# klemens-floege/oneprot

Measured on AMD Instinct MI355X. Metric: protein-pairs/sec/node (seq+struct-token, L=512, ESM-2-150M), higher is better.
Workload: dtype bf16; 1 GPU; cfg-2: seq<->struct_token sub-step, facebook/esm2_t30_150M_UR50D / facebook/esm2_t30_150M_UR50D, L=512, 256 pairs/GPU per modality, global batch 256, output_dim 1024, CLIP local_loss+gather_with_grad, L1 0.01, Adam 1e-3, clip 1.0, sequence encoder frozen (reference default), random-init weights; global_batch=256, seq_len=512, parallelism=dp1, frozen_sequence_encoder=True

## Files before the change

include/oneprot_hip.h:

```cpp
#ifndef ONEPROT_HIP_H
#define ONEPROT_HIP_H
#include <stddef.h>
#include <stdint.h>
#ifdef __cplusplus
extern "C" {
#endif

int oneprot_abi_version(void);

int oneprot_esm_embed_fwd(const int64_t* ids, const float* table, float* x, float* row_scale, int B, int L, int d, int vocab,
                          int pad_id, int mask_id, int token_dropout, void* stream);
size_t oneprot_esm_embed_bwd_workspace(int T, int d, int vocab);
int oneprot_esm_embed_bwd(const int64_t* ids, const float* dx, const float* row_scale, float* dtable, void* workspace, int B, int L, int d,
                          int vocab, int pad_id, int mask_id, int token_dropout, int accumulate, void* stream);
int oneprot_bert_embed_fwd(const int64_t* ids, const float* word, const float* pos, const float* type0, const float* gamma, const float* beta,
                           float* x_f32, void* x_bf16, int B, int L, int d, int vocab, float eps, void* stream);

int oneprot_layernorm_fwd(const void* x, int x_is_bf16, const float* gamma, const float* beta, void* y_bf16, float* y_f32, float* mean,
                          float* rstd, int64_t T, int d, float eps, void* stream);
size_t oneprot_layernorm_bwd_workspace(int d);
int oneprot_layernorm_bwd(const void* dy, int dy_mode, const float* wrow, int L, const void* x, int x_is_bf16, const float* gamma,
                          const float* mean, const float* rstd, const float* add_to, float* dx, void* dx_bf16 ,
                          float* dgamma, float* dbeta, void* workspace, int64_t T, int d, int accumulate_param_grads, void* stream);
int oneprot_lnpool_fwd(const float* x, const int64_t* ids, int pad_id, const float* gamma, const float* beta, float* pooled, float* mean,
                       float* rstd, float* wrow, void* hidden_bf16, float* hidden_f32, int B, int L, int d, float eps, int mode, void* stream);

int oneprot_pool_fwd(const float* x, const int64_t* ids, int pad_id, float* pooled, int B, int L, int d, int mode, void* stream);
int oneprot_pool_bwd(const float* dpooled, const int64_t* ids, int pad_id, float* g, void* g_bf16, int B, int L, int d, int mode, void* stream);
int oneprot_embed_scatter_sorted(const float* dx, const int64_t* perm, const int64_t* seg_start, const int64_t* seg_row, int64_t n_tokens, int n_seg,
                                 int d, int skip_row, float* dtable, void* stream);
int oneprot_rowsum_f32(const float* x, float* out, int R, int64_t n, void* stream);

int oneprot_attnpool_fwd(const float* x, const int64_t* ids, int pad_id, const float* w, const float* bias, float* pooled, float* attn, int B, int L,
                         int d, void* stream);
size_t oneprot_attnpool_bwd_workspace(int B, int d);
int oneprot_attnpool_bwd(const float* x, const float* attn, const float* w, const float* dpooled, float* dw, float* db, float* dx, void* workspace,
                         int B, int L, int d, void* stream);

enum {
  ONEPROT_EPI_BF16 = 0,
  ONEPROT_EPI_F32 = 1,
  ONEPROT_EPI_BIAS_GELU = 2,
  ONEPROT_EPI_BIAS_RESID = 3,
  ONEPROT_EPI_QKV_ROPE = 4,
  ONEPROT_EPI_GELU_BWD = 5
};
int oneprot_gemm_bf16_nt(const void* A, const void* Bw, int64_t M, int N, int K, int lda, int ldb, int epilogue, const float* bias,
                         void* out0, void* out1, void* out2, const void* aux, const float* rope_cos, const float* rope_sin, float q_scale,
                         int L, int H, int hd, void* stream);
int oneprot_gemm_ln_pack_weight(const void* W_bf16 , void* Wp, int N, int K, void* stream);
int oneprot_gemm_bf16_nt_resid_ln(const void* A, const void* Wp, int64_t M, int N, int K, int lda, const float* bias, const float* resid, float* x_out,
                                  const float* gamma, const float* beta, float eps, void* h_out, float* mean, float* rstd, void* stream);
size_t oneprot_sched_workspace_bytes(int64_t M_max);
int oneprot_alloc_uncached(void** out, size_t bytes);
int oneprot_free_uncached(void* ptr);
int oneprot_sched_workspace_init(void* sched_ws, size_t bytes, void* stream);
void oneprot_dynamic_tiles(void* sched_ws, size_t bytes);
int oneprot_sched_late_draws(const void* sched_ws);
int64_t oneprot_sched_epoch(const void* sched_ws);
int oneprot_gemm_resid_ln8_eligible(int64_t M, int N, int K);
int oneprot_gemm_resid_ln8_error(const void* sched_ws);
int oneprot_gemm_resid_ln8_error_clear(void* sched_ws, void* stream);
void oneprot_gemm_resid_ln8_poll_bound(int polls);
int oneprot_gemm_bf16_nt_resid_ln8(const void* A, const void* W, int64_t M, int N, int K, int lda, int ldb, const float* bias, const float* resid,
                                   float* x_out, const float* gamma, const float* beta, float eps, void* h_bf16, float* stats, void* sched_ws,
                                   size_t sched_ws_bytes, void* stream);
void oneprot_gemm_ln_form(int form);
int oneprot_gemm_ln_form_get(void);
void oneprot_gemm_force_shape(int shape);
void oneprot_gemm_tune(int sup_m, int sup_n);
size_t oneprot_gemm_bf16_tn_workspace(int N, int K);
void oneprot_gemm_tn_variant(int v);
void oneprot_cu_reserve(int cus);
int oneprot_gemm_bf16_tn(const void* dY, const void* X, int64_t M, int N, int K, int ldy, int ldx, float* dW, float* dbias, void* workspace,
                         size_t workspace_bytes, int accumulate, void* stream);
int oneprot_sgemm(const float* A, const float* B, float* C, int M, int N, int K, int transA, int b_is_kn, float alpha, int accumulate, void* stream);

int oneprot_attn_fwd(const void* q, const void* k, const void* v, const float* key_bias, void* ctx, float* lse, int B, int H, int L, int hd,
                     void* stream);
size_t oneprot_attn_bwd_workspace(int B, int H, int L);
int oneprot_attn_bwd(const void* q, const void* k, const void* v, const float* key_bias, const void* ctx, const void* dctx, const float* lse,
                     const float* rope_cos, const float* rope_sin, float q_scale, void* dqkv, void* workspace, int B, int H, int L, int hd,
                     void* stream);
int oneprot_attn_fwd_dropout(const void* q, const void* k, const void* v, const float* key_bias, void* ctx, float* lse, int B, int H, int L, int hd,
                             float p, uint64_t seed, uint64_t stream_id, void* stream);
int oneprot_attn_bwd_dropout(const void* q, const void* k, const void* v, const float* key_bias, const void* ctx, const void* dctx, const float* lse,
                             const float* rope_cos, const float* rope_sin, float q_scale, void* dqkv, void* workspace, int B, int H, int L, int hd,
                             float p, uint64_t seed, uint64_t stream_id, void* stream);
int oneprot_attn_dropout_keep(void* keep, int B, int H, int L, float p, uint64_t seed, uint64_t stream_id, void* stream);
void oneprot_attn_force_bwd_path(int path);
void oneprot_attn_force_fwd_path(int path);

int oneprot_gelu_f32(const float* x, float* y, int64_t n, void* stream);
int oneprot_gelu_bwd_f32(const float* x, const float* dy, float* dx, int64_t n, void* stream);
int oneprot_l2norm_fwd(const float* x, float* y, float* inv_norm, int R, int D, float scale, void* stream);
int oneprot_l2norm_bwd(const float* y, const float* dy, const float* inv_norm, float* dx, int R, int D, float scale, float l1_coef, void* stream);
int oneprot_ce_fwd_bwd(float* logits, float* loss_sum, float* row_loss_ws , int R, int C, int label_offset, float row_weight, void* stream);
int oneprot_siglip_fwd_bwd(float* logits, float* loss_sum, float* row_loss_ws , int B, float logit_bias, int negative_only, void* stream);
int oneprot_siglip_fwd_bwd_dev(float* logits, float* loss_sum, float* row_loss_ws , int B, const float* logit_bias_dev, int negative_only, void* stream);
int oneprot_diag_rank(const float* logits, int* rank_row, int* rank_col, int N, void* stream);
int oneprot_abs_sum(const float* x, float* out_sum, void* workspace , int64_t n, float coef, void* stream);

int oneprot_dot_f32(const float* x, const float* y, float* out_sum, void* workspace , int64_t n, float coef, void* stream);

int oneprot_l1_bwd(const float* x, float* dx, int64_t n, float coef, const float* upstream, int accumulate, void* stream);
int oneprot_scale_by_device_scalar(float* x, int64_t n, const float* s, void* stream);
int oneprot_key_padding_bias(const int64_t* ids, float* bias, int64_t n, int pad_id, void* stream);

int oneprot_dropout_bf16(const void* x, void* y, int64_t n, float p, uint64_t seed, uint64_t stream_id, void* stream);
int oneprot_dropout_f32(const float* x, float* y, int64_t n, float p, uint64_t seed, uint64_t stream_id, void* stream);
int oneprot_dropout_add_f32(const float* x, const float* resid, float* y, int64_t n, float p, uint64_t seed, uint64_t stream_id, void* stream);
int oneprot_dropout_add_layernorm_fwd(const float* x, const float* resid, float* s_out, const float* gamma, const float* beta, void* y_bf16, float* y_f32,
                                      float* mean, float* rstd, int64_t T, int d, float eps, float p, uint64_t seed, uint64_t stream_id, void* stream);
int oneprot_dropout_bwd_add_bf16(const void* dy, void* dx, int64_t n, float p, uint64_t seed, uint64_t stream_id, void* stream);
int oneprot_dropout_bwd_add_f32(const void* dy, float* dx, int64_t n, float p, uint64_t seed, uint64_t stream_id, void* stream);

size_t oneprot_sumsq_workspace(void);
int oneprot_sumsq(const float* x, int64_t n, float* sumsq, void* workspace, void* stream);
int oneprot_clip_coef(const float* sumsq, float max_norm, float* coef, float* norm_out, const void* sched_ws , void* stream);
int oneprot_adam_step(float* p, const float* g, float* m, float* v, int64_t n, float lr, float beta1, float beta2, float eps, float weight_decay,
                      int step, const float* grad_scale, void* stream);

int oneprot_cast_f32_to_bf16(const float* src, void* dst, int64_t n, void* stream);
int oneprot_transpose_cast_f32_to_bf16(const float* src, void* dst, int R, int C, void* stream);
int oneprot_transpose_cast_f32_to_bf16_batched(const float* src, void* dst, int R, int C, int64_t src_stride, int64_t dst_stride, int count, void* stream);
size_t oneprot_colsum_workspace(int N);
// ... 28 lines not shown
```

oneprot_amd/csrc/gemm_tn.hip:

```cpp
#include "common.h"
#include "../../include/oneprot_hip.h"

#define TN_MAX_SLAB_TILES 512

static __device__ __attribute__((aligned(16))) unsigned int g_zero_page[4] = {0, 0, 0, 0};

__device__ __forceinline__ int tn_f(int r) { return 2 * ((r & 3) | (((r >> 3) & 1) << 2)); }

__device__ __forceinline__ bf8_t tn_frag(const unsigned char* tile, int mb, int c0, int lane) {
  const int g = lane >> 4, i = lane & 15;
  const int r0 = mb + 8 * g + (i >> 2), r1 = r0 + 4;
  const int col = c0 + 4 * (i & 3);
  const int chunk = col >> 3, within = (col & 7) * 2;
  const unsigned char* p0 = tile + r0 * 256 + ((chunk ^ tn_f(r0)) << 4) + within;
  const unsigned char* p1 = tile + r1 * 256 + ((chunk ^ tn_f(r1)) << 4) + within;
  const s16x4 a = __builtin_amdgcn_ds_read_tr16_b64_v4i16((__attribute__((address_space(3))) s16x4*)p0);
  const s16x4 b = __builtin_amdgcn_ds_read_tr16_b64_v4i16((__attribute__((address_space(3))) s16x4*)p1);
  s16x8 o;
  o[0] = a[0]; o[1] = a[1]; o[2] = a[2]; o[3] = a[3]; o[4] = b[0]; o[5] = b[1]; o[6] = b[2]; o[7] = b[3];
  return __builtin_bit_cast(bf8_t, o);
}

template <int N> __device__ __forceinline__ void tn_wait_vmcnt() { asm volatile("s_waitcnt vmcnt(%0)" ::"n"(N) : "memory"); }

template <int BT, int NSTAGE, int MINW, bool RS>
__global__ void __launch_bounds__(256, MINW) k_gemm_tn(const bf16_t* __restrict__ dY, const bf16_t* __restrict__ X, int M, int N, int K, int ldy, int ldx,
                                                       float* __restrict__ slab, float* __restrict__ bias_slab, int tiles_k, int tiles_all, int S, int m_per_split) {
  constexpr int TILE_BYTES = BT * 256;
  constexpr int STAGE_BYTES = 2 * TILE_BYTES;
  constexpr int IPW = BT / 4 / 4;
  constexpr int LPS = 2 * IPW;
  extern __shared__ __attribute__((aligned(16))) unsigned char smem[];
  const int per_xcd = gridDim.x >> 3;
  const int xcd = blockIdx.x & 7, seq = blockIdx.x >> 3;
  const int w = xcd * per_xcd + seq;
  if (w >= tiles_all * S) return;
  const int split = w / tiles_all, tile = w - split * tiles_all;
  const int tn = tile / tiles_k, tk = tile - tn * tiles_k;
  const int n0 = tn * 128, k0 = tk * 128;
  const int tid = threadIdx.x, lane = tid & 63;
  const int wave = __builtin_amdgcn_readfirstlane(tid >> 6);
  const int wr = wave >> 1, wc = wave & 1;
  const int mbeg = split * m_per_split;
  const int mend = min(M, mbeg + m_per_split);
  const int nsteps = (mend - mbeg + BT - 1) / BT;

  const int srow = lane >> 4, schunk = lane & 15;
  const unsigned char* zero = reinterpret_cast<const unsigned char*>(g_zero_page);
  int rows[IPW], ycol_ok[IPW], xcol_ok[IPW];
  size_t yoff[IPW], xoff[IPW];
#pragma unroll
  for (int i = 0; i < IPW; ++i) {
    rows[i] = (wave * IPW + i) * 4 + srow;
    const int sc = schunk ^ tn_f(rows[i]);
// ... 157 lines not shown
        if (n < N) bias_slab[(size_t)split * N + n] = accb[i][r];
      }
  }
}

__global__ void __launch_bounds__(256) k_tn_reduce(const float* __restrict__ slab, float* __restrict__ dW, size_t n4, size_t stride4, int S, int accumulate,
                                                   const float* __restrict__ bias_slab, float* __restrict__ db, int N, int bias_blocks) {
  const int wblocks = (int)gridDim.x - bias_blocks;
  if ((int)blockIdx.x >= wblocks) {
    const int n = ((int)blockIdx.x - wblocks) * 256 + threadIdx.x;
    if (n >= N) return;
    float s = 0.f;
    for (int p = 0; p < S; ++p) s += bias_slab[(size_t)p * N + n];
    db[n] = accumulate ? db[n] + s : s;
    return;
  }
  for (size_t i = (size_t)blockIdx.x * 256 + threadIdx.x; i < n4; i += (size_t)wblocks * 256) {
    float4 s = reinterpret_cast<const float4*>(slab)[i];
    for (int p = 1; p < S; ++p) {
      const float4 v = reinterpret_cast<const float4*>(slab)[i + (size_t)p * stride4];
      s.x += v.x; s.y += v.y; s.z += v.z; s.w += v.w;
    }
    if (accumulate) { const float4 o = reinterpret_cast<const float4*>(dW)[i]; s.x += o.x; s.y += o.y; s.z += o.z; s.w += o.w; }
    reinterpret_cast<float4*>(dW)[i] = s;
  }
}

__device__ __forceinline__ int tn_f640(int r) { return 2 * (((r >> 1) & 1) | (((r >> 3) & 1) << 1)); }
template <int PITCH> __device__ __forceinline__ int tn8_swz(int r) { return PITCH == 640 ? tn_f640(r) : tn_f(r); }

__device__ __forceinline__ void tn8_glds16(unsigned voff, const unsigned char* sbase, unsigned lds_dst) {
  unsigned keep;
  asm volatile("s_mov_b32 %0, m0\n\ts_mov_b32 m0, %3\n\ts_nop 0\n\tglobal_load_lds_dwordx4 %1, %2\n\ts_mov_b32 m0, %0"
               : "=&s"(keep) : "v"(voff), "s"(sbase), "s"(lds_dst) : "memory");
}
__device__ __forceinline__ bf8_t tn8_frag(const unsigned char* p0, const unsigned char* p1) {
  const s16x4 a = __builtin_amdgcn_ds_read_tr16_b64_v4i16((__attribute__((address_space(3))) s16x4*)p0);
  const s16x4 b = __builtin_amdgcn_ds_read_tr16_b64_v4i16((__attribute__((address_space(3))) s16x4*)p1);
  s16x8 o;
  o[0] = a[0]; o[1] = a[1]; o[2] = a[2]; o[3] = a[3]; o[4] = b[0]; o[5] = b[1]; o[6] = b[2]; o[7] = b[3];
  return __builtin_bit_cast(bf8_t, o);
}

#ifdef TN8_STAMP
static __device__ unsigned long long g_tn8_stamps[2 * 64 * 8];
extern "C" int oneprot_tn8_debug_read(unsigned long long* dst) { return hipMemcpyFromSymbol(dst, HIP_SYMBOL(g_tn8_stamps), sizeof(g_tn8_stamps)) == hipSuccess ? 0 : -2; }
#define TN8_ST(i) do { if (blockIdx.x == 0 && (wave & 3) == 0 && p < 64) { unsigned long long t_; asm volatile("s_memtime %0\n\ts_waitcnt lgkmcnt(0)" : "=s"(t_) :: "memory"); \
    if (lane == 0) g_tn8_stamps[(grp * 64 + p) * 8 + (i)] = t_; } } while (0)
#else
#define TN8_ST(i) do { } while (0)
#endif
#define TN8_RING 4

template <int YC, int XC>
__global__ void __launch_bounds__(512, 2) k_gemm_tn8(const bf16_t* __restrict__ dY, const bf16_t* __restrict__ X, int M, int N, int K, int ldy, int ldx,
                                                     float* __restrict__ slab, float* __restrict__ bias_slab, int tiles_k, int tiles_all, int S) {
  constexpr int MT = YC / 64, NT = XC / 32;
  constexpr int PY = YC * 2, PX = XC * 2;
  constexpr int UY = 32 * PY, UX = 32 * PX, UNIT = UY + UX;
  constexpr int YP = UY / 1024, NP = UNIT / 1024;
  constexpr int IPW = (NP + 7) / 8;
  constexpr int NBY = PY == 640 ? 1 : 2, NBX = PX == 640 ? 2 : 4;
  static_assert(MT * NT == 40 && NP == 36 && IPW == 5, "tile");
  extern __shared__ __attribute__((aligned(16))) unsigned char smem[];
  const int per_xcd = gridDim.x >> 3;
  const int xcd = blockIdx.x & 7, seq = blockIdx.x >> 3;
  const int w = xcd * per_xcd + seq;
  if (w >= tiles_all * S) return;
  const int split = w / tiles_all, tile = w - split * tiles_all;
  const int tn = tile / tiles_k, tk = tile - tn * tiles_k;
  const int n0 = tn * YC, k0 = tk * XC;
  const int tid = threadIdx.x, lane = tid & 63;
  const int wave = __builtin_amdgcn_readfirstlane(tid >> 6);
  const int grp = wave >> 2;
  const int wn = wave >> 1, wk = wave & 1;
  const int units = M >> 5, ubase = units / S, urem = units - ubase * S;
  const int P = ubase + (split < urem ? 1 : 0);
  const int u0 = split * ubase + (split < urem ? split : urem);
  const unsigned lds0 = (unsigned)(uintptr_t)LDS_PTR(smem);

  unsigned voff[IPW]; unsigned pdst[IPW]; bool isy[IPW];
#pragma unroll
  for (int i = 0; i < IPW; ++i) {
    const int piece = i * 8 + wave;
    isy[i] = piece < YP;
    if (isy[i]) {
      const int idx = piece * 64 + lane, row = idx / (PY / 16), pos = idx - row * (PY / 16);
      int col = n0 + (pos ^ tn8_swz<PY>(row)) * 8;
      if (col >= N) col -= 256;
      voff[i] = (unsigned)row * (unsigned)ldy * 2u + (unsigned)col * 2u;
      pdst[i] = piece * 1024;
    } else {
      const int idx = (piece - YP) * 64 + lane, row = idx / (PX / 16), pos = idx - row * (PX / 16);
      voff[i] = (unsigned)row * (unsigned)ldx * 2u + (unsigned)(k0 + (pos ^ tn8_swz<PX>(row)) * 8) * 2u;
      pdst[i] = UY + (piece - YP) * 1024;
    }
  }
  const unsigned char* ybase = reinterpret_cast<const unsigned char*>(dY + (size_t)u0 * 32 * ldy);
  const unsigned char* xbase = reinterpret_cast<const unsigned char*>(X + (size_t)u0 * 32 * ldx);
  const size_t ystep = (size_t)32 * ldy * 2, xstep = (size_t)32 * ldx * 2;
  auto issue = [&](int u, int slot) {
    const unsigned char* yb = ybase + (size_t)u * ystep;
    const unsigned char* xb = xbase + (size_t)u * xstep;
    const unsigned dst = lds0 + slot * UNIT;
#pragma unroll
    for (int i = 0; i < IPW; ++i)
      if (i + 1 < IPW || wave < 4) tn8_glds16(voff[i], isy[i] ? yb : xb, dst + pdst[i]);
  };

  const int g = lane >> 4, i16 = lane & 15;
  const int rr[2] = {8 * g + (i16 >> 2), 8 * g + (i16 >> 2) + 4};
  const int within = (i16 & 1) * 8, cb = (i16 & 3) >> 1;
  unsigned yb_[NBY][2], xb_[NBX][2];
#pragma unroll
  for (int rd = 0; rd < 2; ++rd) {
#pragma unroll
    for (int k = 0; k < NBY; ++k)
      yb_[k][rd] = rr[rd] * PY + (((k * 8 + 2 * wn + cb) ^ tn8_swz<PY>(rr[rd])) << 4) + within - k * 128;
#pragma unroll
    for (int k = 0; k < NBX; ++k)
      xb_[k][rd] = UY + rr[rd] * PX + (((k * 4 + 2 * wk + cb) ^ tn8_swz<PX>(rr[rd])) << 4) + within - k * 64;
  }

  f32x4 acc[MT][NT], accb[MT];
  {
    float z = 0.f;
    asm volatile("" : "+v"(z));
#pragma unroll
    for (int i = 0; i < MT; ++i) {
      accb[i] = (f32x4){z, z, z, z};
#pragma unroll
      for (int j = 0; j < NT; ++j) acc[i][j] = (f32x4){z, z, z, z};
    }
  }
  const bool do_bias = bias_slab != nullptr && tk == 0 && wk == 0;
  const u32x4 ones_u = {0x3F803F80u, 0x3F803F80u, 0x3F803F80u, 0x3F803F80u};
  const bf8_t ones = __builtin_bit_cast(bf8_t, ones_u);

#pragma unroll
  for (int u = 0; u < 3; ++u)
    if (u < P) issue(u, u);
  if (P > 2) { if (grp == 0) tn_wait_vmcnt<2 * IPW>(); else tn_wait_vmcnt<2 * (IPW - 1)>(); }
  else tn_wait_vmcnt<0>();
  asm volatile("s_barrier" ::: "memory");
  if (grp == 1) asm volatile("s_barrier" ::: "memory");

  int slot = 0, nslot = 3;
#pragma clang loop unroll(disable)
  for (int p = 0; p < P; ++p) {
    const unsigned char* ub = smem + slot * UNIT;
    bf8_t fa[MT], fb[NT];
#pragma unroll
    for (int i = 0; i < MT; ++i) fa[i] = tn8_frag(ub + yb_[i % NBY][0] + i * 128, ub + yb_[i % NBY][1] + i * 128);
#pragma unroll
    for (int j = 0; j < NT; ++j) fb[j] = tn8_frag(ub + xb_[j % NBX][0] + j * 64, ub + xb_[j % NBX][1] + j * 64);
    __builtin_amdgcn_sched_barrier(0);
    TN8_ST(2);
    const bool more = p + 3 < P;
    asm volatile("s_waitcnt lgkmcnt(0)" ::: "memory");
    TN8_ST(4);
    if (p + 2 < P) { if (grp == 0) tn_wait_vmcnt<IPW>(); else tn_wait_vmcnt<IPW - 1>(); }
    else tn_wait_vmcnt<0>();
    TN8_ST(5);
    asm volatile("s_barrier" ::: "memory");
    TN8_ST(0);
    __builtin_amdgcn_sched_barrier(0);
    __builtin_amdgcn_s_setprio(1);
#pragma unroll
    for (int i = 0; i < MT; ++i) {
#pragma unroll
      for (int j = 0; j < NT; ++j) acc[i][j] = __builtin_amdgcn_mfma_f32_16x16x32_bf16(fa[i], fb[j], acc[i][j], 0, 0, 0);
      if (i == 0) {
        __builtin_amdgcn_sched_barrier(0);
        if (more) issue(p + 3, nslot);
        __builtin_amdgcn_sched_barrier(0);
      }
    }
    TN8_ST(3);
    if (do_bias) {
#pragma unroll
      for (int i = 0; i < MT; ++i) accb[i] = __builtin_amdgcn_mfma_f32_16x16x32_bf16(fa[i], ones, accb[i], 0, 0, 0);
    }
    __builtin_amdgcn_s_setprio(0);
    __builtin_amdgcn_sched_barrier(0);
    TN8_ST(6);
    asm volatile("s_barrier" ::: "memory");
    TN8_ST(1);
    slot = slot + 1 == TN8_RING ? 0 : slot + 1;
    nslot = nslot + 1 == TN8_RING ? 0 : nslot + 1;
  }
  if (grp == 0) asm volatile("s_barrier" ::: "memory");

  float* out = slab + (size_t)split * N * K;
  const int fq = lane >> 4, fr = lane & 15;
#pragma unroll
  for (int i = 0; i < MT; ++i)
#pragma unroll
    for (int r = 0; r < 4; ++r) {
      const int n = n0 + (4 * i + wn) * 16 + fq * 4 + r;
      if (n < N) {
#pragma unroll
        for (int j = 0; j < NT; ++j) out[(size_t)n * K + k0 + (2 * j + wk) * 16 + fr] = acc[i][j][r];
      }
    }
  if (do_bias && fr == 0) {
#pragma unroll
    for (int i = 0; i < MT; ++i)
#pragma unroll
      for (int r = 0; r < 4; ++r) {
        const int n = n0 + (4 * i + wn) * 16 + fq * 4 + r;
        if (n < N) bias_slab[(size_t)split * N + n] = accb[i][r];
      }
  }
}

static int tn8_config(int N, int K) {
  if (K % 320 == 0 && N % 256 == 0) return 1;
  if (N % 320 == 0 && K % 256 == 0) return 2;
  if (K % 320 == 0 && N >= 256 && N % 64 == 0) return 1;
  return 0;
}
static int tn8_tiles(int cfg, int N, int K) { return cfg == 1 ? ((N + 255) / 256) * (K / 320) : (N / 320) * (K / 256); }
static int g_cu_reserve = 0;
extern "C" void oneprot_cu_reserve(int cus) { g_cu_reserve = cus < 0 ? 0 : cus; }
static int tn8_cus_all() {
  static int n_cu = 0;
  if (n_cu == 0) {
    int dev = 0; hipDeviceProp_t prop;
    n_cu = (hipGetDevice(&dev) == hipSuccess && hipGetDeviceProperties(&prop, dev) == hipSuccess && prop.multiProcessorCount > 0) ? prop.multiProcessorCount : 256;
  }
  return n_cu;
}
static int tn8_cus() {
  const int n = tn8_cus_all() - g_cu_reserve;
  return n < 64 ? 64 : n;
}
static int tn8_splits(int64_t M, int tiles, int n_cu, int64_t max_by_workspace) {
  if (M % 32) return 0;
  int S = n_cu / tiles;
  if (S > 64) S = 64;
  if (S > M / 256) S = (int)(M / 256);
  if (S > max_by_workspace) S = (int)max_by_workspace;
  if (S < 1 || (int64_t)S * tiles * 2 < n_cu) return 0;
  return S;
}

static int g_tn_variant = -1;
extern "C" void oneprot_gemm_tn_variant(int v) { g_tn_variant = v; }

static inline int tn_splits(int64_t M, int tiles) {
  int S = TN_MAX_SLAB_TILES / tiles;
  if (S < 1) S = 1;
  const int64_t max_by_m = (M + 255) / 256;
  if (M > 0 && S > max_by_m) S = (int)max_by_m;
  if (S > 64) S = 64;
  return S;
}

extern "C" size_t oneprot_gemm_bf16_tn_workspace(int N, int K) {
  const int tiles = ((N + 127) / 128) * ((K + 127) / 128);
  int S = tn_splits(0, tiles);
  const int cfg = tn8_config(N, K);
  if (cfg) {
    int S8 = tn8_cus_all() / tn8_tiles(cfg, N, K);
    if (S8 > 64) S8 = 64;
    if (S8 > S) S = S8;
  }
  return (size_t)S * N * K * sizeof(float) + (size_t)S * N * sizeof(float);
}

extern "C" int oneprot_gemm_bf16_tn(const void* dY, const void* X, int64_t M, int N, int K, int ldy, int ldx, float* dW, float* dbias, void* workspace,
                                    size_t workspace_bytes, int accumulate, void* stream) {
  if (!dY || !X || !dW || !workspace || M <= 0 || N <= 0 || K <= 0 || M > 0x7fffffff) return OP_EINVAL;
  if ((N & 7) || (K & 7) || (ldy & 7) || (ldx & 7) || ldy < N || ldx < K || ((N * (int64_t)K) & 3)) return OP_EINVAL;
  if (((uintptr_t)dY | (uintptr_t)X | (uintptr_t)dW | (uintptr_t)workspace) & 15) return OP_EINVAL;
  const int variant = (g_tn_variant < 0 || g_tn_variant == 3) ? 2 : g_tn_variant;
  hipStream_t s = (hipStream_t)stream;
  if (g_tn_variant < 0 || g_tn_variant == 3) {
    const int cfg = tn8_config(N, K);
    if (cfg && (size_t)32 * ldy * 2 < (1u << 31) && (size_t)32 * ldx * 2 < (1u << 31)) {
      const int tiles8 = tn8_tiles(cfg, N, K);
      const size_t per_split = (size_t)N * K * sizeof(float) + (dbias ? (size_t)N * sizeof(float) : 0);
      const int S8 = tn8_splits(M, tiles8, tn8_cus(), 64);
      if (S8 > 0 && workspace_bytes < (size_t)S8 * per_split) return OP_EINVAL;
      if (S8 > 0) {
        constexpr int LDS8 = TN8_RING * 36 * 1024;
        static bool c8 = false;
        if (!c8) {
          if (hipFuncSetAttribute((const void*)k_gemm_tn8<256, 320>, hipFuncAttributeMaxDynamicSharedMemorySize, LDS8) != hipSuccess) return OP_ELAUNCH;
          if (hipFuncSetAttribute((const void*)k_gemm_tn8<320, 256>, hipFuncAttributeMaxDynamicSharedMemorySize, LDS8) != hipSuccess) return OP_ELAUNCH;
          c8 = true;
        }
        const int tiles_k8 = cfg == 1 ? K / 320 : K / 256;
        float* bias_slab8 = dbias ? (float*)workspace + (size_t)S8 * N * K : nullptr;
        const dim3 grid(8 * ((tiles8 * S8 + 7) / 8));
        if (cfg == 1) hipLaunchKernelGGL((k_gemm_tn8<256, 320>), grid, dim3(512), LDS8, s, (const bf16_t*)dY, (const bf16_t*)X, (int)M, N, K, ldy, ldx, (float*)workspace, bias_slab8, tiles_k8, tiles8, S8);
        else hipLaunchKernelGGL((k_gemm_tn8<320, 256>), grid, dim3(512), LDS8, s, (const bf16_t*)dY, (const bf16_t*)X, (int)M, N, K, ldy, ldx, (float*)workspace, bias_slab8, tiles_k8, tiles8, S8);
        const size_t n4_8 = ((size_t)N * K) >> 2;
        size_t blocks8 = (n4_8 + 255) / 256; if (blocks8 > 4096) blocks8 = 4096;
        const int bb8 = dbias ? (N + 255) / 256 : 0;
        hipLaunchKernelGGL(k_tn_reduce, dim3((unsigned)blocks8 + bb8), dim3(256), 0, s, (const float*)workspace, dW, n4_8, n4_8, S8, accumulate, (const float*)bias_slab8, dbias, N, bb8);
        return launch_status();
      }
    }
  }
  const int tiles_n = (N + 127) / 128, tiles_k = (K + 127) / 128, tiles = tiles_n * tiles_k;
  const int S = tn_splits(M, tiles);
  if (workspace_bytes < (size_t)S * N * K * sizeof(float) + (dbias ? (size_t)S * N * sizeof(float) : 0)) return OP_EINVAL;
  float* bias_slab = dbias ? (float*)workspace + (size_t)S * N * K : nullptr;
  const int BT = variant == 1 ? 32 : 64;
  int m_per = (int)((M + S - 1) / S);
  m_per = ((m_per + BT - 1) / BT) * BT;
  if (variant == 0) {
    static bool c0 = false;
    if (!c0) { if (hipFuncSetAttribute((const void*)k_gemm_tn<64, 2, 2, false>, hipFuncAttributeMaxDynamicSharedMemorySize, 2 * 2 * 64 * 256) != hipSuccess) return OP_ELAUNCH; c0 = true; }
    hipLaunchKernelGGL((k_gemm_tn<64, 2, 2, false>), dim3(8 * ((tiles * S + 7) / 8)), dim3(256), 2 * 2 * 64 * 256, s, (const bf16_t*)dY, (const bf16_t*)X, (int)M, N, K, ldy, ldx,
                       (float*)workspace, bias_slab, tiles_k, tiles, S, m_per);
  } else if (variant == 2) {
    static bool c2 = false;
    if (!c2) { if (hipFuncSetAttribute((const void*)k_gemm_tn<64, 2, 2, true>, hipFuncAttributeMaxDynamicSharedMemorySize, 2 * 2 * 64 * 256) != hipSuccess) return OP_ELAUNCH; c2 = true; }
    hipLaunchKernelGGL((k_gemm_tn<64, 2, 2, true>), dim3(8 * ((tiles * S + 7) / 8)), dim3(256), 2 * 2 * 64 * 256, s, (const bf16_t*)dY, (const bf16_t*)X, (int)M, N, K, ldy, ldx,
                       (float*)workspace, bias_slab, tiles_k, tiles, S, m_per);
  } else {
    static bool c1 = false;
    if (!c1) { if (hipFuncSetAttribute((const void*)k_gemm_tn<32, 3, 3, false>, hipFuncAttributeMaxDynamicSharedMemorySize, 3 * 2 * 32 * 256) != hipSuccess) return OP_ELAUNCH; c1 = true; }
    hipLaunchKernelGGL((k_gemm_tn<32, 3, 3, false>), dim3(8 * ((tiles * S + 7) / 8)), dim3(256), 3 * 2 * 32 * 256, s, (const bf16_t*)dY, (const bf16_t*)X, (int)M, N, K, ldy, ldx,
                       (float*)workspace, bias_slab, tiles_k, tiles, S, m_per);
  }
  const size_t n4 = ((size_t)N * K) >> 2;
  size_t blocks = (n4 + 255) / 256; if (blocks > 4096) blocks = 4096;
  const int bb = dbias ? (N + 255) / 256 : 0;
  hipLaunchKernelGGL(k_tn_reduce, dim3((unsigned)blocks + bb), dim3(256), 0, s, (const float*)workspace, dW, n4, n4, S, accumulate, (const float*)bias_slab, dbias, N, bb);
  return launch_status();
}
```

oneprot_amd/hip.py:

```python
import ctypes
import os
from ctypes import c_float, c_int, c_int64, c_size_t, c_void_p

import torch

_HERE = os.path.dirname(os.path.abspath(__file__))
LIB_PATH = os.environ.get("ONEPROT_HIP_LIB") or os.path.join(_HERE, "liboneprot_hip.so")

ABI_VERSION = 7
EPI_BF16, EPI_F32, EPI_BIAS_GELU, EPI_BIAS_RESID, EPI_QKV_ROPE, EPI_GELU_BWD = range(6)
LOG2E = 1.4426950408889634


class HipLibraryMissing(RuntimeError):
    pass


class HipKernelError(RuntimeError):
    pass


P, I, L64, F, SZ = c_void_p, c_int, c_int64, c_float, c_size_t
U64 = ctypes.c_uint64

_SIGS = {
    "oneprot_abi_version": (I, []),
    "oneprot_esm_embed_fwd": (I, [P, P, P, P, I, I, I, I, I, I, I, P]),
    "oneprot_esm_embed_bwd_workspace": (SZ, [I, I, I]),
    "oneprot_esm_embed_bwd": (I, [P, P, P, P, P, I, I, I, I, I, I, I, I, P]),
    "oneprot_bert_embed_fwd": (I, [P, P, P, P, P, P, P, P, I, I, I, I, F, P]),
    "oneprot_pool_fwd": (I, [P, P, I, P, I, I, I, I, P]),
    "oneprot_pool_bwd": (I, [P, P, I, P, P, I, I, I, I, P]),
    "oneprot_embed_scatter_sorted": (I, [P, P, P, P, L64, I, I, I, P, P]),
    "oneprot_rowsum_f32": (I, [P, P, I, L64, P]),
    "oneprot_attnpool_fwd": (I, [P, P, I, P, P, P, P, I, I, I, P]),
    "oneprot_attnpool_bwd_workspace": (SZ, [I, I]),
    "oneprot_attnpool_bwd": (I, [P, P, P, P, P, P, P, P, I, I, I, P]),
    "oneprot_layernorm_fwd": (I, [P, I, P, P, P, P, P, P, L64, I, F, P]),
    "oneprot_layernorm_bwd_workspace": (SZ, [I]),
    "oneprot_layernorm_bwd": (I, [P, I, P, I, P, I, P, P, P, P, P, P, P, P, P, L64, I, I, P]),
    "oneprot_lnpool_fwd": (I, [P, P, I, P, P, P, P, P, P, P, P, I, I, I, F, I, P]),
    "oneprot_gemm_bf16_nt": (I, [P, P, L64, I, I, I, I, I, P, P, P, P, P, P, P, F, I, I, I, P]),
    "oneprot_gemm_ln_pack_weight": (I, [P, P, I, I, P]),
    "oneprot_gemm_bf16_nt_resid_ln": (I, [P, P, L64, I, I, I, P, P, P, P, P, F, P, P, P, P]),
    "oneprot_sched_workspace_bytes": (SZ, [L64]),
    "oneprot_alloc_uncached": (I, [ctypes.POINTER(c_void_p), SZ]),
    "oneprot_free_uncached": (I, [P]),
    "oneprot_sched_workspace_init": (I, [P, SZ, P]),
    "oneprot_dynamic_tiles": (None, [P, SZ]),
    "oneprot_sched_late_draws": (I, [P]),
    "oneprot_sched_epoch": (L64, [P]),
    "oneprot_gemm_bf16_nt_resid_ln8": (I, [P, P, L64, I, I, I, I, P, P, P, P, P, F, P, P, P, SZ, P]),
    "oneprot_gemm_resid_ln8_eligible": (I, [L64, I, I]),
    "oneprot_gemm_resid_ln8_error": (I, [P]),
    "oneprot_gemm_resid_ln8_error_clear": (I, [P, P]),
    "oneprot_gemm_resid_ln8_poll_bound": (None, [I]),
    "oneprot_gemm_ln_form": (None, [I]),
    "oneprot_gemm_ln_form_get": (I, []),
    "oneprot_gemm_force_shape": (None, [I]),
    "oneprot_gemm_tune": (None, [I, I]),
    "oneprot_gemm_bf16_tn_workspace": (SZ, [I, I]),
    "oneprot_gemm_tn_variant": (None, [I]),
    "oneprot_cu_reserve": (None, [I]),
    "oneprot_gemm_bf16_tn": (I, [P, P, L64, I, I, I, I, P, P, P, SZ, I, P]),
    "oneprot_sgemm": (I, [P, P, P, I, I, I, I, I, F, I, P]),
    "oneprot_attn_fwd": (I, [P, P, P, P, P, P, I, I, I, I, P]),
    "oneprot_attn_fwd_dropout": (I, [P, P, P, P, P, P, I, I, I, I, F, U64, U64, P]),
    "oneprot_attn_dropout_keep": (I, [P, I, I, I, F, U64, U64, P]),
    "oneprot_attn_bwd_dropout": (I, [P, P, P, P, P, P, P, P, P, F, P, P, I, I, I, I, F, U64, U64, P]),
    "oneprot_attn_bwd_workspace": (SZ, [I, I, I]),
    "oneprot_attn_bwd": (I, [P, P, P, P, P, P, P, P, P, F, P, P, I, I, I, I, P]),
    "oneprot_attn_force_bwd_path": (None, [I]),
    "oneprot_attn_force_fwd_path": (None, [I]),
    "oneprot_gelu_f32": (I, [P, P, L64, P]),
    "oneprot_gelu_bwd_f32": (I, [P, P, P, L64, P]),
    "oneprot_l2norm_fwd": (I, [P, P, P, I, I, F, P]),
    "oneprot_l2norm_bwd": (I, [P, P, P, P, I, I, F, F, P]),
    "oneprot_ce_fwd_bwd": (I, [P, P, P, I, I, I, F, P]),
    "oneprot_siglip_fwd_bwd": (I, [P, P, P, I, F, I, P]),
    "oneprot_siglip_fwd_bwd_dev": (I, [P, P, P, I, P, I, P]),
    "oneprot_diag_rank": (I, [P, P, P, I, P]),
    "oneprot_abs_sum": (I, [P, P, P, L64, F, P]),
    "oneprot_dot_f32": (I, [P, P, P, P, L64, F, P]),
    "oneprot_l1_bwd": (I, [P, P, L64, F, P, I, P]),
    "oneprot_scale_by_device_scalar": (I, [P, L64, P, P]),
    "oneprot_dropout_bf16": (I, [P, P, L64, F, U64, U64, P]),
    "oneprot_dropout_bwd_add_bf16": (I, [P, P, L64, F, U64, U64, P]),
    "oneprot_dropout_bwd_add_f32": (I, [P, P, L64, F, U64, U64, P]),
    "oneprot_dropout_f32": (I, [P, P, L64, F, U64, U64, P]),
    "oneprot_dropout_add_f32": (I, [P, P, P, L64, F, U64, U64, P]),
    "oneprot_dropout_add_layernorm_fwd": (I, [P, P, P, P, P, P, P, P, P, L64, I, F, F, U64, U64, P]),
    "oneprot_key_padding_bias": (I, [P, P, L64, I, P]),
    "oneprot_sumsq_workspace": (SZ, []),
    "oneprot_sumsq": (I, [P, L64, P, P, P]),
    "oneprot_clip_coef": (I, [P, F, P, P, P, P]),
    "oneprot_adam_step": (I, [P, P, P, P, L64, F, F, F, F, F, I, P, P]),
    "oneprot_cast_f32_to_bf16": (I, [P, P, L64, P]),
    "oneprot_transpose_cast_f32_to_bf16": (I, [P, P, I, I, P]),
    "oneprot_transpose_cast_f32_to_bf16_batched": (I, [P, P, I, I, L64, L64, I, P]),
    "oneprot_colsum_workspace": (SZ, [I]),
    "oneprot_colsum_bf16": (I, [P, P, P, L64, I, I, P]),
    "oneprot_esm_embed_packed_fwd": (I, [P, P, P, P, P, P, P, P, P, I, I, I, I, I, I, I, I, I, I, P]),
    "oneprot_esm_embed_packed_bwd": (I, [P, P, P, P, P, I, I, I, I, I, I, I, P]),
    "oneprot_attn_varlen_fwd": (I, [P, P, P, P, P, I, P, P, I, I, I, I, P]),
    "oneprot_attn_varlen_bwd_workspace": (SZ, [I, I]),
    "oneprot_attn_varlen_bwd": (I, [P, P, P, P, P, I, P, P, P, P, P, F, P, P, I, I, I, I, P]),
    "oneprot_lnpool_packed_fwd": (I, [P, P, P, I, P, P, P, P, P, P, P, I, I, I, F, I, P]),
    "oneprot_lnpool_packed_bwd": (I, [P, P, P, P, P, P, P, P, P, P, P, P, I, I, I, P]),
    "oneprot_attnpool_packed_fwd": (I, [P, P, P, I, P, P, P, P, I, I, I, P]),
    "oneprot_attnpool_packed_bwd": (I, [P, P, P, P, P, P, P, P, P, I, I, I, I, P]),
}

_PTR_DTYPES = {
    "oneprot_esm_embed_fwd": "lfff", "oneprot_esm_embed_bwd": "lfffb", "oneprot_bert_embed_fwd": "lffffffh", "oneprot_pool_fwd": "flf",
    "oneprot_pool_bwd": "flfh", "oneprot_embed_scatter_sorted": "flllf", "oneprot_rowsum_f32": "ff", "oneprot_attnpool_fwd": "flffff",
    "oneprot_attnpool_bwd": "fffffffb", "oneprot_layernorm_fwd": "*ffhfff", "oneprot_layernorm_bwd": "*f*fffffhffb", "oneprot_lnpool_fwd": "flffffffhf",
# ... 188 lines not shown
```

Measured before the change: 1176 protein-pairs/sec/node.

## Cost-balance split-K work items per tile in TN8 weight-gradient GEMM

Replaces the uniform split-K count in the tn8 weight-gradient GEMM with a host-built, cached plan. Each tile gets its own split count, weighted by a cost model, so short last-row tiles (N not a multiple of 256) get fewer splits. Those partial tiles also run a reduced-MTV kernel body that skips the dead MFMA rows. Work items are sorted and uploaded as a device table, slabs are stored compactly per tile, and a new per-tile reduce kernel replaces the flat one. The aim is to cut load imbalance and wasted compute across CUs, at the cost of more host-side planning complexity and a device item table.

```diff
diff --git a/include/oneprot_hip.h b/include/oneprot_hip.h
--- a/include/oneprot_hip.h
+++ b/include/oneprot_hip.h
@@ -72,6 +72,7 @@
 size_t oneprot_gemm_bf16_tn_workspace(int N, int K);
 void oneprot_gemm_tn_variant(int v);
 void oneprot_cu_reserve(int cus);
+int oneprot_gemm_tn_work_table(int64_t M, int N, int K, int cus, int* items, int max_items);
 int oneprot_gemm_bf16_tn(const void* dY, const void* X, int64_t M, int N, int K, int ldy, int ldx, float* dW, float* dbias, void* workspace,
                          size_t workspace_bytes, int accumulate, void* stream);
 int oneprot_sgemm(const float* A, const float* B, float* C, int M, int N, int K, int transA, int b_is_kn, float alpha, int accumulate, void* stream);
diff --git a/oneprot_amd/csrc/gemm_tn.hip b/oneprot_amd/csrc/gemm_tn.hip
--- a/oneprot_amd/csrc/gemm_tn.hip
+++ b/oneprot_amd/csrc/gemm_tn.hip
@@ -1,5 +1,9 @@
 #include "common.h"
 #include "../../include/oneprot_hip.h"
+#include <algorithm>
+#include <mutex>
+#include <utility>
+#include <vector>
 
 #define TN_MAX_SLAB_TILES 512
 
@@ -263,31 +267,21 @@
 #endif
 #define TN8_RING 4
 
-template <int YC, int XC>
-__global__ void __launch_bounds__(512, 2) k_gemm_tn8(const bf16_t* __restrict__ dY, const bf16_t* __restrict__ X, int M, int N, int K, int ldy, int ldx,
-                                                     float* __restrict__ slab, float* __restrict__ bias_slab, int tiles_k, int tiles_all, int S) {
+template <int YC, int XC, int MTV>
+__device__ __forceinline__ void tn8_body(unsigned char* smem, const bf16_t* __restrict__ dY, const bf16_t* __restrict__ X, int ldy, int ldx, int n0, int k0, int u0, int P,
+                                         float* __restrict__ out, float* __restrict__ bout) {
   constexpr int MT = YC / 64, NT = XC / 32;
-  constexpr int PY = YC * 2, PX = XC * 2;
+  constexpr int YS = (MTV < MT && MTV <= 2) ? 128 : YC;
+  constexpr int PY = YS * 2, PX = XC * 2;
   constexpr int UY = 32 * PY, UX = 32 * PX, UNIT = UY + UX;
   constexpr int YP = UY / 1024, NP = UNIT / 1024;
   constexpr int IPW = (NP + 7) / 8;
   constexpr int NBY = PY == 640 ? 1 : 2, NBX = PX == 640 ? 2 : 4;
-  static_assert(MT * NT == 40 && NP == 36 && IPW == 5, "tile");
-  extern __shared__ __attribute__((aligned(16))) unsigned char smem[];
-  const int per_xcd = gridDim.x >> 3;
-  const int xcd = blockIdx.x & 7, seq = blockIdx.x >> 3;
-  const int w = xcd * per_xcd + seq;
-  if (w >= tiles_all * S) return;
-  const int split = w / tiles_all, tile = w - split * tiles_all;
-  const int tn = tile / tiles_k, tk = tile - tn * tiles_k;
-  const int n0 = tn * YC, k0 = tk * XC;
+  static_assert(MT * NT == 40 && (NP == 36 || NP == 28) && NP % 8 == 4 && MTV >= 1 && MTV <= MT && (MTV == MT || YC == 256), "tile");
   const int tid = threadIdx.x, lane = tid & 63;
   const int wave = __builtin_amdgcn_readfirstlane(tid >> 6);
   const int grp = wave >> 2;
   const int wn = wave >> 1, wk = wave & 1;
-  const int units = M >> 5, ubase = units / S, urem = units - ubase * S;
-  const int P = ubase + (split < urem ? 1 : 0);
-  const int u0 = split * ubase + (split < urem ? split : urem);
   const unsigned lds0 = (unsigned)(uintptr_t)LDS_PTR(smem);
 
   unsigned voff[IPW]; unsigned pdst[IPW]; bool isy[IPW];
@@ -297,9 +291,9 @@
     isy[i] = piece < YP;
     if (isy[i]) {
       const int idx = piece * 64 + lane, row = idx / (PY / 16), pos = idx - row * (PY / 16);
-      int col = n0 + (pos ^ tn8_swz<PY>(row)) * 8;
-      if (col >= N) col -= 256;
-      voff[i] = (unsigned)row * (unsigned)ldy * 2u + (unsigned)col * 2u;
+      int col = (pos ^ tn8_swz<PY>(row)) * 8;
+      if (YS > MTV * 64 && col >= MTV * 64) col -= 64;
+      voff[i] = (unsigned)row * (unsigned)ldy * 2u + (unsigned)(n0 + col) * 2u;
       pdst[i] = piece * 1024;
     } else {
       const int idx = (piece - YP) * 64 + lane, row = idx / (PX / 16), pos = idx - row * (PX / 16);
@@ -333,18 +327,18 @@
       xb_[k][rd] = UY + rr[rd] * PX + (((k * 4 + 2 * wk + cb) ^ tn8_swz<PX>(rr[rd])) << 4) + within - k * 64;
   }
 
-  f32x4 acc[MT][NT], accb[MT];
+  f32x4 acc[MTV][NT], accb[MTV];
   {
     float z = 0.f;
     asm volatile("" : "+v"(z));
 #pragma unroll
-    for (int i = 0; i < MT; ++i) {
+    for (int i = 0; i < MTV; ++i) {
       accb[i] = (f32x4){z, z, z, z};
 #pragma unroll
       for (int j = 0; j < NT; ++j) acc[i][j] = (f32x4){z, z, z, z};
     }
   }
-  const bool do_bias = bias_slab != nullptr && tk == 0 && wk == 0;
+  const bool do_bias = bout != nullptr && wk == 0;
   const u32x4 ones_u = {0x3F803F80u, 0x3F803F80u, 0x3F803F80u, 0x3F803F80u};
   const bf8_t ones = __builtin_bit_cast(bf8_t, ones_u);
 
@@ -360,9 +354,9 @@
 #pragma clang loop unroll(disable)
   for (int p = 0; p < P; ++p) {
     const unsigned char* ub = smem + slot * UNIT;
-    bf8_t fa[MT], fb[NT];
-#pragma unroll
-    for (int i = 0; i < MT; ++i) fa[i] = tn8_frag(ub + yb_[i % NBY][0] + i * 128, ub + yb_[i % NBY][1] + i * 128);
+    bf8_t fa[MTV], fb[NT];
+#pragma unroll
+    for (int i = 0; i < MTV; ++i) fa[i] = tn8_frag(ub + yb_[i % NBY][0] + i * 128, ub + yb_[i % NBY][1] + i * 128);
 #pragma unroll
     for (int j = 0; j < NT; ++j) fb[j] = tn8_frag(ub + xb_[j % NBX][0] + j * 64, ub + xb_[j % NBX][1] + j * 64);
     __builtin_amdgcn_sched_barrier(0);
@@ -378,7 +372,7 @@
     __builtin_amdgcn_sched_barrier(0);
     __builtin_amdgcn_s_setprio(1);
 #pragma unroll
-    for (int i = 0; i < MT; ++i) {
+    for (int i = 0; i < MTV; ++i) {
 #pragma unroll
       for (int j = 0; j < NT; ++j) acc[i][j] = __builtin_amdgcn_mfma_f32_16x16x32_bf16(fa[i], fb[j], acc[i][j], 0, 0, 0);
       if (i == 0) {
@@ -390,7 +384,7 @@
     TN8_ST(3);
     if (do_bias) {
 #pragma unroll
-      for (int i = 0; i < MT; ++i) accb[i] = __builtin_amdgcn_mfma_f32_16x16x32_bf16(fa[i], ones, accb[i], 0, 0, 0);
+      for (int i = 0; i < MTV; ++i) accb[i] = __builtin_amdgcn_mfma_f32_16x16x32_bf16(fa[i], ones, accb[i], 0, 0, 0);
     }
     __builtin_amdgcn_s_setprio(0);
     __builtin_amdgcn_sched_barrier(0);
@@ -402,27 +396,84 @@
   }
   if (grp == 0) asm volatile("s_barrier" ::: "memory");
 
-  float* out = slab + (size_t)split * N * K;
   const int fq = lane >> 4, fr = lane & 15;
 #pragma unroll
-  for (int i = 0; i < MT; ++i)
+  for (int i = 0; i < MTV; ++i)
 #pragma unroll
     for (int r = 0; r < 4; ++r) {
-      const int n = n0 + (4 * i + wn) * 16 + fq * 4 + r;
-      if (n < N) {
-#pragma unroll
-        for (int j = 0; j < NT; ++j) out[(size_t)n * K + k0 + (2 * j + wk) * 16 + fr] = acc[i][j][r];
-      }
+      const int n = (4 * i + wn) * 16 + fq * 4 + r;
+#pragma unroll
+      for (int j = 0; j < NT; ++j) out[n * XC + (2 * j + wk) * 16 + fr] = acc[i][j][r];
     }
   if (do_bias && fr == 0) {
 #pragma unroll
-    for (int i = 0; i < MT; ++i)
-#pragma unroll
-      for (int r = 0; r < 4; ++r) {
-        const int n = n0 + (4 * i + wn) * 16 + fq * 4 + r;
-        if (n < N) bias_slab[(size_t)split * N + n] = accb[i][r];
-      }
-  }
+    for (int i = 0; i < MTV; ++i)
+#pragma unroll
+      for (int r = 0; r < 4; ++r) bout[(4 * i + wn) * 16 + fq * 4 + r] = accb[i][r];
+  }
+}
+
+struct Tn8Geo { int tiles_k, n_full, S_full, S_short, rows_short; };
+template <int YC, int XC>
+__host__ __device__ __forceinline__ void tn8_tile(const Tn8Geo& g, int tile, int& n0, int& k0, int& rows, int& S, size_t& soff, int& boff) {
+  const int tn = tile / g.tiles_k, tk = tile - tn * g.tiles_k;
+  const bool sh = tile >= g.n_full;
+  n0 = tn * YC; k0 = tk * XC;
+  rows = sh ? g.rows_short : YC;
+  S = sh ? g.S_short : g.S_full;
+  soff = sh ? (size_t)g.n_full * g.S_full * YC * XC + (size_t)tk * g.S_short * g.rows_short * XC : (size_t)tile * g.S_full * YC * XC;
+  boff = tn * g.S_full * YC;
+}
+template <int YC, int XC, int MTV>
+__global__ void __launch_bounds__(512, 2) k_gemm_tn8(const bf16_t* __restrict__ dY, const bf16_t* __restrict__ X, int M, int ldy, int ldx, float* __restrict__ ws,
+                                                     const unsigned* __restrict__ items, Tn8Geo geo, int n_items, int bias_base) {
+  extern __shared__ __attribute__((aligned(16))) unsigned char smem[];
+  const int per_xcd = gridDim.x >> 3;
+  const int xcd = blockIdx.x & 7, seq = blockIdx.x >> 3;
+  const int w = xcd * per_xcd + seq;
+  if (w >= n_items) return;
+  const unsigned it = items[w];
+  const int tile = it & 0xffff, split = it >> 16;
+  int n0, k0, rows, S, boff; size_t soff;
+  tn8_tile<YC, XC>(geo, tile, n0, k0, rows, S, soff, boff);
+  const int units = M >> 5, ubase = units / S, urem = units - ubase * S;
+  const int P = ubase + (split < urem ? 1 : 0);
+  const int u0 = split * ubase + (split < urem ? split : urem);
+  float* out = ws + soff + (size_t)split * rows * XC;
+  float* bout = (bias_base >= 0 && k0 == 0) ? ws + (size_t)bias_base + boff + split * rows : nullptr;
+  if (MTV == YC / 64 || rows == YC) tn8_body<YC, XC, YC / 64>(smem, dY, X, ldy, ldx, n0, k0, u0, P, out, bout);
+  else tn8_body<YC, XC, MTV>(smem, dY, X, ldy, ldx, n0, k0, u0, P, out, bout);
+}
+
+template <int YC, int XC>
+__global__ void __launch_bounds__(256) k_tn8_reduce(const float* __restrict__ ws, Tn8Geo geo, int n_tiles, float* __restrict__ dW, int K, int accumulate, float* __restrict__ db, int bias_base, int bias_blocks) {
+  constexpr int XC4 = XC / 4, BPT = YC * XC4 / 256;
+  int n0, k0, rows, S, boff; size_t soff;
+  if ((int)blockIdx.x < bias_blocks) {
+    tn8_tile<YC, XC>(geo, (int)blockIdx.x * geo.tiles_k, n0, k0, rows, S, soff, boff);
+    const float* src = ws + (size_t)bias_base + boff;
+    for (int n = threadIdx.x; n < rows; n += 256) {
+      float s = 0.f;
+      for (int p = 0; p < S; ++p) s += src[p * rows + n];
+      db[n0 + n] = accumulate ? db[n0 + n] + s : s;
+    }
+    return;
+  }
+  const int b = (int)blockIdx.x - bias_blocks, tile = b / BPT;
+  if (tile >= n_tiles) return;
+  tn8_tile<YC, XC>(geo, tile, n0, k0, rows, S, soff, boff);
+  const int l = (b - tile * BPT) * 256 + threadIdx.x, area4 = rows * XC4;
+  if (l >= area4) return;
+  const float4* src = reinterpret_cast<const float4*>(ws + soff) + l;
+  float4 s = src[0];
+  for (int p = 1; p < S; ++p) {
+    const float4 v = src[(size_t)p * area4];
+    s.x += v.x; s.y += v.y; s.z += v.z; s.w += v.w;
+  }
+  const int r = l / XC4, c4 = l - r * XC4;
+  float4* dst = reinterpret_cast<float4*>(dW + (size_t)(n0 + r) * K + k0) + c4;
+  if (accumulate) { const float4 o = *dst; s.x += o.x; s.y += o.y; s.z += o.z; s.w += o.w; }
+  *dst = s;
 }
 
 static int tn8_config(int N, int K) {
@@ -431,7 +482,6 @@
   if (K % 320 == 0 && N >= 256 && N % 64 == 0) return 1;
   return 0;
 }
-static int tn8_tiles(int cfg, int N, int K) { return cfg == 1 ? ((N + 255) / 256) * (K / 320) : (N / 320) * (K / 256); }
 static int g_cu_reserve = 0;
 extern "C" void oneprot_cu_reserve(int cus) { g_cu_reserve = cus < 0 ? 0 : cus; }
 static int tn8_cus_all() {
@@ -446,14 +496,111 @@
   const int n = tn8_cus_all() - g_cu_reserve;
   return n < 64 ? 64 : n;
 }
-static int tn8_splits(int64_t M, int tiles, int n_cu, int64_t max_by_workspace) {
-  if (M % 32) return 0;
-  int S = n_cu / tiles;
-  if (S > 64) S = 64;
-  if (S > M / 256) S = (int)(M / 256);
-  if (S > max_by_workspace) S = (int)max_by_workspace;
-  if (S < 1 || (int64_t)S * tiles * 2 < n_cu) return 0;
-  return S;
+#ifndef TN8_FIXED_COST
+#define TN8_FIXED_COST 40
+#endif
+struct Tn8Plan {
+  int cfg = 0, yc = 0, xc = 0, tiles_n = 0, tiles_k = 0, n_tiles = 0, n_items = 0, mtv_last = 0;
+  size_t slab_floats = 0, bias_floats = 0;
+  Tn8Geo geo = {0, 0, 0, 0, 0};
+  std::vector<int> tab;
+  std::vector<unsigned> items;
+};
+static bool tn8_plan(int64_t M, int N, int K, int n_cu, Tn8Plan& p) {
+  p = Tn8Plan();
+  const int cfg = tn8_config(N, K);
+  if (!cfg || M <= 0 || M % 32) return false;
+  const int yc = cfg == 1 ? 256 : 320, xc = cfg == 1 ? 320 : 256;
+  const int tiles_n = (N + yc - 1) / yc, tiles_k = K / xc, nt = tiles_n * tiles_k;
+  const int cap = (int)std::min<int64_t>(64, M / 256);
+  if (cap < 1 || nt > n_cu) return false;
+  std::vector<int> cost(nt), S(nt, 1), rows(nt);
+  for (int t = 0; t < nt; ++t) {
+    rows[t] = std::min(yc, N - (t / tiles_k) * yc);
+    cost[t] = rows[t] == yc ? 400 : 4 * TN8_FIXED_COST + (100 - TN8_FIXED_COST) * (rows[t] / 64);
+  }
+  auto longest = [&]() { int b = 0; for (int t = 1; t < nt; ++t) if ((int64_t)cost[t] * S[b] > (int64_t)cost[b] * S[t]) b = t; return b; };
+  for (int total = nt; total < n_cu; ++total) {
+    const int b = longest();
+    if (S[b] >= cap) break;
+    ++S[b];
+  }
+  const int b = longest();
+  int total = 0;
+  for (int t = 0; t < nt; ++t) { S[t] = (int)(((int64_t)cost[t] * S[b] + cost[b] - 1) / cost[b]); total += S[t]; }
+  if ((int64_t)total * 2 < n_cu) return false;
+  p.cfg = cfg; p.yc = yc; p.xc = xc; p.tiles_n = tiles_n; p.tiles_k = tiles_k; p.n_tiles = nt; p.n_items = total;
+  p.mtv_last = (N - (tiles_n - 1) * yc) / 64;
+  const int n_full = rows[nt - 1] == yc ? nt : nt - tiles_k;
+  p.geo = Tn8Geo{tiles_k, n_full, S[0], S[nt - 1], rows[nt - 1]};
+  p.tab.assign((size_t)8 * nt + 2 * total, 0);
+  std::vector<std::pair<int, int>> items;
+  for (int t = 0; t < nt; ++t) {
+    int n0, k0, rw, St, boff; size_t soff;
+    if (cfg == 1) tn8_tile<256, 320>(p.geo, t, n0, k0, rw, St, soff, boff); else tn8_tile<320, 256>(p.geo, t, n0, k0, rw, St, soff, boff);
+    if (rw != rows[t] || St != S[t]) return false;
+    int* r = &p.tab[8 * t];
+    r[0] = n0; r[1] = k0; r[2] = rw; r[3] = St; r[4] = (int)soff; r[5] = k0 == 0 ? boff : -1;
+    p.slab_floats = std::max(p.slab_floats, soff + (size_t)St * rw * xc);
+    if (k0 == 0) p.bias_floats = std::max(p.bias_floats, (size_t)boff + (size_t)St * rw);
+    for (int sp = 0; sp < St; ++sp) items.emplace_back(t, sp);
+  }
+  std::stable_sort(items.begin(), items.end(), [&](const std::pair<int, int>& x, const std::pair<int, int>& y) {
+    const int64_t l = (int64_t)x.second * S[y.first], r = (int64_t)y.second * S[x.first];
+    return l != r ? l < r : x.first < y.first;
+  });
+  for (int i = 0; i < total; ++i) { p.tab[8 * nt + 2 * i] = items[i].first; p.tab[8 * nt + 2 * i + 1] = items[i].second; p.items.push_back((unsigned)items[i].first | (unsigned)items[i].second << 16); }
+  return true;
+}
+extern "C" int oneprot_gemm_tn_work_table(int64_t M, int N, int K, int cus, int* items, int max_items) {
+  Tn8Plan p;
+  if (N <= 0 || K <= 0 || cus <= 0 || !tn8_plan(M, N, K, cus, p)) return 0;
+  const int units = (int)(M >> 5);
+  for (int i = 0; i < p.n_items && i < max_items && items; ++i) {
+    const int t = p.tab[8 * p.n_tiles + 2 * i], s = p.tab[8 * p.n_tiles + 2 * i + 1];
+    const int* r = &p.tab[8 * t];
+    const int ubase = units / r[3], urem = units - ubase * r[3];
+    int* o = items + 8 * i;
+    o[0] = r[0]; o[1] = r[1]; o[2] = r[2] / 16; o[3] = s * ubase + (s < urem ? s : urem); o[4] = ubase + (s < urem ? 1 : 0);
+    o[5] = r[4] + s * r[2] * p.xc; o[6] = r[2] * p.xc; o[7] = r[5] < 0 ? -1 : (int)p.slab_floats + r[5] + s * r[2];
+  }
+  return p.n_items;
+}
+struct Tn8Cached { int dev, cap, N, K, n_cu; bool ok; Tn8Plan plan; unsigned* d_items; };
+static const Tn8Cached* tn8_table(int64_t M, int N, int K, int n_cu) {
+  static std::mutex mu;
+  static std::vector<Tn8Cached*> cache;
+  int dev = 0;
+  if (hipGetDevice(&dev) != hipSuccess) return nullptr;
+  const int cap = (int)std::min<int64_t>(64, M / 256);
+  std::lock_guard<std::mutex> lock(mu);
+  for (const Tn8Cached* c : cache)
+    if (c->dev == dev && c->cap == cap && c->N == N && c->K == K && c->n_cu == n_cu) return c;
+  Tn8Cached* c = new Tn8Cached{dev, cap, N, K, n_cu, false, Tn8Plan(), nullptr};
+  c->ok = tn8_plan(M, N, K, n_cu, c->plan);
+  if (c->ok) {
+    const size_t bytes = c->plan.items.size() * sizeof(unsigned);
+    if (hipMalloc((void**)&c->d_items, bytes) != hipSuccess || hipMemcpy(c->d_items, c->plan.items.data(), bytes, hipMemcpyHostToDevice) != hipSuccess) { delete c; return nullptr; }
+  }
+  cache.push_back(c);
+  return c;
+}
+template <int YC, int XC, int MTV>
+static int tn8_launch(const Tn8Cached* c, const void* dY, const void* X, int64_t M, int K, int ldy, int ldx, float* dW, float* dbias, void* workspace, int accumulate, hipStream_t s) {
+  constexpr int LDS8 = TN8_RING * 36 * 1024;
+  static bool attr = false;
+  if (!attr) {
+    if (hipFuncSetAttribute((const void*)k_gemm_tn8<YC, XC, MTV>, hipFuncAttributeMaxDynamicSharedMemorySize, LDS8) != hipSuccess) return OP_ELAUNCH;
+    attr = true;
+  }
+  const Tn8Plan& p = c->plan;
+  const int bias_base = dbias ? (int)p.slab_floats : -1;
+  hipLaunchKernelGGL((k_gemm_tn8<YC, XC, MTV>), dim3(8 * ((p.n_items + 7) / 8)), dim3(512), LDS8, s, (const bf16_t*)dY, (const bf16_t*)X, (int)M, ldy, ldx, (float*)workspace,
+                     (const unsigned*)c->d_items, p.geo, p.n_items, bias_base);
+  constexpr int bpt = YC * XC / 4 / 256;
+  const int bb = dbias ? p.tiles_n : 0;
+  hipLaunchKernelGGL((k_tn8_reduce<YC, XC>), dim3(p.n_tiles * bpt + bb), dim3(256), 0, s, (const float*)workspace, p.geo, p.n_tiles, dW, K, accumulate, dbias, bias_base, bb);
+  return launch_status();
 }
 
 static int g_tn_variant = -1;
@@ -472,12 +619,12 @@
   const int tiles = ((N + 127) / 128) * ((K + 127) / 128);
   int S = tn_splits(0, tiles);
   const int cfg = tn8_config(N, K);
+  size_t need = (size_t)S * N * K * sizeof(float) + (size_t)S * N * sizeof(float);
   if (cfg) {
-    int S8 = tn8_cus_all() / tn8_tiles(cfg, N, K);
-    if (S8 > 64) S8 = 64;
-    if (S8 > S) S = S8;
-  }
-  return (size_t)S * N * K * sizeof(float) + (size_t)S * N * sizeof(float);
+    const size_t yc = cfg == 1 ? 256 : 320, xc = cfg == 1 ? 320 : 256;
+    need = std::max(need, (size_t)tn8_cus_all() * (yc * xc + yc) * sizeof(float));
+  }
+  return need;
 }
 
 extern "C" int oneprot_gemm_bf16_tn(const void* dY, const void* X, int64_t M, int N, int K, int ldy, int ldx, float* dW, float* dbias, void* workspace,
@@ -489,29 +636,19 @@
   hipStream_t s = (hipStream_t)stream;
   if (g_tn_variant < 0 || g_tn_variant == 3) {
     const int cfg = tn8_config(N, K);
-    if (cfg && (size_t)32 * ldy * 2 < (1u << 31) && (size_t)32 * ldx * 2 < (1u << 31)) {
-      const int tiles8 = tn8_tiles(cfg, N, K);
-      const size_t per_split = (size_t)N * K * sizeof(float) + (dbias ? (size_t)N * sizeof(float) : 0);
-      const int S8 = tn8_splits(M, tiles8, tn8_cus(), 64);
-      if (S8 > 0 && workspace_bytes < (size_t)S8 * per_split) return OP_EINVAL;
-      if (S8 > 0) {
-        constexpr int LDS8 = TN8_RING * 36 * 1024;
-        static bool c8 = false;
-        if (!c8) {
-          if (hipFuncSetAttribute((const void*)k_gemm_tn8<256, 320>, hipFuncAttributeMaxDynamicSharedMemorySize, LDS8) != hipSuccess) return OP_ELAUNCH;
-          if (hipFuncSetAttribute((const void*)k_gemm_tn8<320, 256>, hipFuncAttributeMaxDynamicSharedMemorySize, LDS8) != hipSuccess) return OP_ELAUNCH;
-          c8 = true;
+    if (cfg && M % 32 == 0 && (size_t)32 * ldy * 2 < (1u << 31) && (size_t)32 * ldx * 2 < (1u << 31)) {
+      const Tn8Cached* c = tn8_table(M, N, K, tn8_cus());
+      if (!c) return OP_ELAUNCH;
+      if (c->ok) {
+        const Tn8Plan& p = c->plan;
+        if (workspace_bytes < (p.slab_floats + (dbias ? p.bias_floats : 0)) * sizeof(float)) return OP_EINVAL;
+        if (cfg == 2) return tn8_launch<320, 256, 5>(c, dY, X, M, K, ldy, ldx, dW, dbias, workspace, accumulate, s);
+        switch (p.mtv_last) {
+          case 1: return tn8_launch<256, 320, 1>(c, dY, X, M, K, ldy, ldx, dW, dbias, workspace, accumulate, s);
+          case 2: return tn8_launch<256, 320, 2>(c, dY, X, M, K, ldy, ldx, dW, dbias, workspace, accumulate, s);
+          case 3: return tn8_launch<256, 320, 3>(c, dY, X, M, K, ldy, ldx, dW, dbias, workspace, accumulate, s);
+          default: return tn8_launch<256, 320, 4>(c, dY, X, M, K, ldy, ldx, dW, dbias, workspace, accumulate, s);
         }
-        const int tiles_k8 = cfg == 1 ? K / 320 : K / 256;
-        float* bias_slab8 = dbias ? (float*)workspace + (size_t)S8 * N * K : nullptr;
-        const dim3 grid(8 * ((tiles8 * S8 + 7) / 8));
-        if (cfg == 1) hipLaunchKernelGGL((k_gemm_tn8<256, 320>), grid, dim3(512), LDS8, s, (const bf16_t*)dY, (const bf16_t*)X, (int)M, N, K, ldy, ldx, (float*)workspace, bias_slab8, tiles_k8, tiles8, S8);
-        else hipLaunchKernelGGL((k_gemm_tn8<320, 256>), grid, dim3(512), LDS8, s, (const bf16_t*)dY, (const bf16_t*)X, (int)M, N, K, ldy, ldx, (float*)workspace, bias_slab8, tiles_k8, tiles8, S8);
-        const size_t n4_8 = ((size_t)N * K) >> 2;
-        size_t blocks8 = (n4_8 + 255) / 256; if (blocks8 > 4096) blocks8 = 4096;
-        const int bb8 = dbias ? (N + 255) / 256 : 0;
-        hipLaunchKernelGGL(k_tn_reduce, dim3((unsigned)blocks8 + bb8), dim3(256), 0, s, (const float*)workspace, dW, n4_8, n4_8, S8, accumulate, (const float*)bias_slab8, dbias, N, bb8);
-        return launch_status();
       }
     }
   }
diff --git a/oneprot_amd/hip.py b/oneprot_amd/hip.py
--- a/oneprot_amd/hip.py
+++ b/oneprot_amd/hip.py
@@ -62,6 +62,7 @@
     "oneprot_gemm_bf16_tn_workspace": (SZ, [I, I]),
     "oneprot_gemm_tn_variant": (None, [I]),
     "oneprot_cu_reserve": (None, [I]),
+    "oneprot_gemm_tn_work_table": (I, [L64, I, I, I, P, I]),
     "oneprot_gemm_bf16_tn": (I, [P, P, L64, I, I, I, I, P, P, P, SZ, I, P]),
     "oneprot_sgemm": (I, [P, P, P, I, I, I, I, I, F, I, P]),
     "oneprot_attn_fwd": (I, [P, P, P, P, P, P, I, I, I, I, P]),
```

After: 1177 protein-pairs/sec/node (median of 2 runs). Within noise of the previous version (+0.0%).
